# alguoo314/JASPER

Measured on AMD Instinct MI355X. Metric: assembly Mbp/s polished + Gk-mers/s counted, k=37, higher is better.
Workload: dtype u64

## Files before the change

jasper_amd/csrc/count_part.hip:

```cpp
#include "table.hpp"
#include <algorithm>
#include <cmath>
#include <cstdio>
#include <cstdlib>
#include <type_traits>
#include <vector>

namespace jk {

#define HIPCHK(x)                                                                     \
    do {                                                                              \
        hipError_t e_ = (x);                                                          \
        if (e_ != hipSuccess) {                                                       \
            err = std::string(#x) + ": " + hipGetErrorString(e_);                     \
            return -1;                                                                \
        }                                                                             \
    } while (0)

__device__ __forceinline__ void lds_barrier() { asm volatile("s_waitcnt lgkmcnt(0)\n\ts_barrier" ::: "memory"); }

constexpr int PT_THREADS = 1024;
constexpr int PT_GROUP = 16;
constexpr int PT_TILE = PT_THREADS * PT_GROUP;
constexpr int PT_HALO = 4;
// ... 686 lines not shown
                uint32_t b2;
                if constexpr (OWN) {
                    b2 = G.p2 ? (uint32_t)(rec[j] >> shift2) & ((1u << G.p2) - 1u) : 0u;
                    b2 |= owner_of(hash_of(b1, rec[j], G.recbits), nown) << G.p2;
                } else b2 = (uint32_t)(rec[j] >> shift2) & (uint32_t)(nb2 - 1);
                br[j] = (b2 << 16) | (atomicAdd(&s_cnt[b2], 1u) & 0xFFFFu);
            }
            lds_barrier();
            {
                const unsigned int v0 = 2 * t < nb2 ? s_cnt[2 * t] : 0u, v1 = 2 * t + 1 < nb2 ? s_cnt[2 * t + 1] : 0u;
                const unsigned int v = v0 + v1;
                unsigned int inc = v;
#pragma unroll
                for (int o = 1; o < 64; o <<= 1) { const unsigned int u = __shfl_up(inc, o); if ((t & 63) >= o) inc += u; }
                if ((t & 63) == 63) s_wsum[t >> 6] = inc;
                lds_barrier();
                unsigned int wbase = 0;
                for (int w = 0; w < (t >> 6); ++w) wbase += s_wsum[w];
                const unsigned int ex = wbase + inc - v;
                if (2 * t < nb2) s_off[2 * t] = ex;
                if (2 * t + 1 < nb2) s_off[2 * t + 1] = ex + v0;
                if (t == PT_THREADS - 1) s_off[nb2] = wbase + inc;
            }
            lds_barrier();
#pragma unroll
            for (int j = 0; j < PT_GROUP; ++j)
                if (br[j] != 0xFFFFFFFFu) s_stage[s_off[br[j] >> 16] + (br[j] & 0xFFFFu)] = rec[j];
            lds_barrier();
            {
                const int lpb = nb2 <= 256 ? 64 : 16;
                const int g = t / lpb, r = t % lpb;
                for (int b2 = g; b2 < nb2; b2 += PT_THREADS / lpb) {
                    const unsigned int off = s_off[b2], cnt = s_cnt[b2], cur = s_cur[b2];
                    const uint64_t region = OWN ? ((((uint64_t)(b2 >> G.p2) << G.p1) + b1) << G.p2) + (uint64_t)(b2 & ((1 << G.p2) - 1))
                                                : ((uint64_t)b1 << G.p2) + (uint64_t)b2;
                    uint64_t *dst = out2 + (region * G.nblk2 + blockIdx.x) * G.cap2;
                    for (unsigned int q = r; q < cnt; q += lpb) {
                        const unsigned int pos = cur + q;
                        const uint64_t rr = s_stage[off + q];
                        if (pos < G.cap2) dst[pos] = rr;
                        else if (MIN && cbits) {
                            const u128 hh = hash_of(b1, rr & ((1ull << G.recbits) - 1ull), G.recbits);
                            const unsigned long long di = atomicAdd(deferred_n, 1ull);
                            if (di < deferred_cap) { deferred[3 * di] = hh.hi; deferred[3 * di + 1] = hh.lo; deferred[3 * di + 2] = ((rr >> G.recbits) & ((1ull << cbits) - 1ull)) + 1ull; }
                            else atomicExch(&T.stats[ST_FATAL], 1ull);
                        } else defer_record(T, hash_of(b1, rr, G.recbits), deferred, deferred_n, deferred_cap);
                    }
                }
            }
            lds_barrier();
            for (int i = t; i < nb2; i += PT_THREADS) { s_cur[i] += s_cnt[i]; s_cnt[i] = 0; }
            lds_barrier();
        }
        for (int i = t; i < nb2; i += PT_THREADS) {
            const uint64_t region = OWN ? ((((uint64_t)(i >> G.p2) << G.p1) + b1) << G.p2) + (uint64_t)(i & ((1 << G.p2) - 1)) : ((uint64_t)b1 << G.p2) + (uint64_t)i;
            cnt2[region * G.nblk2 + blockIdx.x] = s_cur[i] < G.cap2 ? s_cur[i] : G.cap2;
        }
        lds_barrier();
    }
}
constexpr size_t P2_LDS = (size_t)PT_TILE * 8 + (size_t)(3 * PT_MAXBUCKETS + 1 + 16 + P2_MAXSL + 1) * 4;

constexpr int P2F_LINE = 16;
struct P2Meta { uint64_t gbase; uint32_t lim; int32_t cadd; };
__device__ __forceinline__ u128 rec_hash(uint64_t b1, uint64_t r, int recbits) { return hash_of(b1, r, recbits); }
__device__ __forceinline__ u128 rec_hash(uint64_t b1, Rec16 r, int recbits) { return hash_of16(b1, r, recbits); }
template <int MAXB, int ROWS, int RB = 8> struct P2F {
    static constexpr int TILE = PT_THREADS * ROWS;
    static constexpr int PIECE = 64 * ROWS * 9;
    static constexpr size_t LDS = (size_t)TILE * RB + (size_t)(3 * (MAXB + 4) + 32) * 4 + (size_t)MAXB * sizeof(P2Meta) + (size_t)MAXB * 128;
};
struct P2Args {
    int p1, p2, recbits;
    uint32_t nblk1, vper, nblk2, cap1, cap2;
    uint32_t nown;
    unsigned long long *stats;
};
template <int MAXB, int ROWS, bool OWN = false, typename REC = uint64_t>
__global__ __launch_bounds__(PT_THREADS, 4) void part2f_kernel(const REC *__restrict__ out1, const unsigned int *__restrict__ cnt1, P2Args P, REC *__restrict__ out2,
                                                            unsigned int *__restrict__ cnt2, unsigned long long *__restrict__ deferred,
                                                            unsigned long long *__restrict__ deferred_n, uint64_t deferred_cap) {
    constexpr int P2F_MAXB = MAXB, P2F_ROWS = ROWS, P2F_PIECE = P2F<MAXB, ROWS>::PIECE;
    constexpr bool W16 = sizeof(REC) == 16;
    constexpr int RB = (int)sizeof(REC), P2F_LINE = 128 / RB;
    typedef __attribute__((address_space(1))) REC global_rec;
    constexpr int NSW = MAXB / 64;
    extern __shared__ __align__(16) unsigned char s_raw[];
    P2Meta *s_meta = reinterpret_cast<P2Meta *>(s_raw);
    REC *s_carry = reinterpret_cast<REC *>(s_meta + P2F_MAXB);
    unsigned int *s_cnt = reinterpret_cast<unsigned int *>(s_carry + P2F_MAXB * P2F_LINE);
    unsigned int *s_off = s_cnt + P2F_MAXB + 4;
    unsigned int *s_have = s_off + P2F_MAXB + 4;
    unsigned int *s_wsum = s_have + P2F_MAXB + 4;
    REC *s_stage = reinterpret_cast<REC *>(s_wsum + 32);
    const int t = threadIdx.x;
    const int nb2 = OWN ? (int)(P.nown << P.p2) : 1 << P.p2;
    const int shift2 = P.recbits - P.p2;
    const uint32_t wave = (uint32_t)__builtin_amdgcn_readfirstlane(t >> 6), lane = (uint32_t)t & 63u;
    for (uint32_t b1 = blockIdx.y; b1 < (1u << P.p1); b1 += gridDim.y) {
        auto list_of = [&](uint32_t b2) -> uint64_t {
            if constexpr (OWN) return ((((uint64_t)(b2 >> P.p2) << P.p1) + b1) << P.p2) + (uint64_t)(b2 & ((1u << P.p2) - 1u));
            else return ((uint64_t)b1 << P.p2) + (uint64_t)b2;
        };
        auto b2_of = [&](REC rr) -> uint32_t {
            if constexpr (W16) return (uint32_t)shr(mk(rr.hi, rr.lo), (unsigned)shift2).lo & (uint32_t)(nb2 - 1);
            else if constexpr (OWN) {
                const uint32_t lo = P.p2 ? (uint32_t)(rr >> shift2) & ((1u << P.p2) - 1u) : 0u;
                return lo | (owner_of(hash_of(b1, rr, P.recbits), P.nown) << P.p2);
            } else return (uint32_t)(rr >> shift2) & (uint32_t)(nb2 - 1);
        };
        auto slice_of = [&](uint32_t b2) { return reinterpret_cast<uint64_t>(out2 + (list_of(b2) * P.nblk2 + blockIdx.x) * P.cap2); };
        if (t < P2F_MAXB + 4) s_cnt[t] = 0;
        if (t == 0) { s_wsum[16] = 0; s_wsum[17] = 0; }
        static_assert(P2F_MAXB + 4 <= PT_THREADS && NSW >= 1 && NSW <= 16, "list counts are scanned by the first MAXB / 64 waves");
        lds_barrier();
        auto piece_len = [&](uint32_t ph_, uint32_t sub_) -> uint32_t {
            const uint32_t c = cnt1[((uint64_t)ph_ << P.p1) + b1], first = sub_ * (uint32_t)P2F_PIECE;
            return c > first ? (c - first < (uint32_t)P2F_PIECE ? c - first : (uint32_t)P2F_PIECE) : 0u;
        };
        {
            uint32_t rounds = 0;
            for (uint32_t q = wave + 16u * lane;; q += 16u * 64u) {
                const uint32_t ph_ = blockIdx.x + P.nblk2 * (q / P.vper);
                if (ph_ >= P.nblk1) break;
                rounds += (piece_len(ph_, q % P.vper) + 64u * P2F_ROWS - 1u) / (64u * P2F_ROWS);
            }
            for (int o = 32; o > 0; o >>= 1) rounds += __shfl_xor(rounds, o);
            if (lane == 0) atomicMax(&s_wsum[17], rounds);
        }
        lds_barrier();
        const uint32_t rounds = s_wsum[17];
        uint32_t pos = 0;
        uint32_t ph = blockIdx.x + P.nblk2 * (wave / P.vper), sub = wave % P.vper;
        auto open_piece = [&](uint32_t &len_out, const REC *&src_out) {
            len_out = 0;
            if (ph < P.nblk1) {
                const uint32_t c = (uint32_t)__builtin_amdgcn_readfirstlane((int)cnt1[((uint64_t)ph << P.p1) + b1]), first = sub * (uint32_t)P2F_PIECE;
                len_out = c > first ? (c - first < (uint32_t)P2F_PIECE ? c - first : (uint32_t)P2F_PIECE) : 0u;
            }
            src_out = out1 + ((uint64_t)b1 * P.nblk1 + ph) * P.cap1 + (uint64_t)sub * P2F_PIECE;
        };
        uint32_t slen;
        const REC *src;
        open_piece(slen, src);
        unsigned int cur = 0, have = 0;
        REC rec[P2F_ROWS];
        auto fetch = [&](REC (&dst)[P2F_ROWS], uint32_t &valid) {
            while (pos >= slen && ph < P.nblk1) {
                sub += 16u;
                while (sub >= P.vper) { sub -= P.vper; ph += P.nblk2; }
                pos = 0;
                open_piece(slen, src);
            }
            valid = 0;
#pragma unroll
            for (int j = 0; j < P2F_ROWS; ++j) {
                const uint32_t i = pos + (uint32_t)j * 64u + lane;
                if constexpr (W16) { dst[j].lo = ~0ull; dst[j].hi = ~0ull; } else dst[j] = ~0ull;
                if (i < slen) { dst[j] = src[i]; valid |= 1u << j; }
            }
            pos += 64u * P2F_ROWS;
        };
        uint32_t vmask = 0;
        constexpr bool PF = true;
        REC nxt[P2F_ROWS];
        uint32_t vmask_n = 0;
        if (PF && rounds) {
            fetch(rec, vmask);
#pragma unroll
            for (int j = 0; j < P2F_ROWS; ++j) { if constexpr (W16) asm volatile("" : "+v"(rec[j].lo), "+v"(rec[j].hi)); else asm volatile("" : "+v"(rec[j])); }
        }
        for (uint32_t round = 0; round < rounds; ++round) {
            if constexpr (PF) { if (round + 1 < rounds) fetch(nxt, vmask_n); else vmask_n = 0; }
            else fetch(rec, vmask);
            uint32_t br[P2F_ROWS];
#pragma unroll
            for (int j = 0; j < P2F_ROWS; ++j) {
                const uint32_t b2 = (vmask >> j) & 1u ? b2_of(rec[j]) : (uint32_t)nb2;
                br[j] = (b2 << 16) | (atomicAdd(&s_cnt[b2], 1u) & 0xFFFFu);
            }
            lds_barrier();
            unsigned int v = 0, inc = 0;
            if (t < P2F_MAXB) {
                v = t < nb2 ? s_cnt[t] : 0u;
                inc = wave_scan_incl(v);
                if (lane == 63) s_wsum[wave] = inc;
                s_cnt[t] = 0;
                if (t == 0) s_cnt[nb2] = 0;
            }
            lds_barrier();
            unsigned int total, wbase;
            if constexpr (NSW == 2) { total = s_wsum[0] + s_wsum[1]; wbase = wave ? s_wsum[0] : 0u; }
            else {
                const unsigned int ws = wave_scan_incl(lane < (uint32_t)NSW ? s_wsum[lane] : 0u);
                wbase = wave && wave < (uint32_t)NSW ? (unsigned int)__builtin_amdgcn_readlane((int)ws, (int)wave - 1) : 0u;
                total = (unsigned int)__builtin_amdgcn_readlane((int)ws, NSW - 1);
            }
            unsigned int F = 0;
            if (t < nb2) {
                const unsigned int ex = inc - v + wbase;
                const unsigned int T = have + v;
                F = T & ~(unsigned int)(P2F_LINE - 1);
                const unsigned int L = F ? F - have : 0u;
                s_off[t] = ex;
                P2Meta M;
                M.gbase = slice_of((uint32_t)t) + ((uint64_t)cur + (uint64_t)have - (uint64_t)ex) * (uint64_t)RB;
                M.lim = ex + L;
                M.cadd = F ? -(int32_t)(ex + L) : (int32_t)have - (int32_t)ex;
                s_meta[t] = M;
                s_have[t] = have | (F ? 0x80000000u : 0u);
                if (cur + F > P.cap2) s_wsum[16] = 1;
            }
            if (t == 0) s_off[nb2] = total;
            lds_barrier();
#pragma unroll
            for (int j = 0; j < P2F_ROWS; ++j) s_stage[s_off[br[j] >> 16] + (br[j] & 0xFFFFu)] = rec[j];
            int td = t;
            asm volatile("" : "+v"(td));
            constexpr int NU = P2F_MAXB / 64;
            REC cw[NU];
            uint32_t cat[NU];
#pragma unroll
            for (int u = 0; u < NU; ++u) {
                if constexpr (W16) { cw[u].lo = 0ull; cw[u].hi = 0ull; } else cw[u] = 0ull;
                cat[u] = ~0u;
                const uint32_t b2 = ((uint32_t)td >> 4) + (uint32_t)u * 64u, q = (uint32_t)td & 15u;
                if (b2 < (uint32_t)nb2) {
                    const unsigned int hv = s_have[b2];
                    if ((hv >> 31) && q < (hv & 0xFFFFu)) {
                        cw[u] = s_carry[b2 * P2F_LINE + q];
                        const P2Meta M = s_meta[b2];
                        cat[u] = (uint32_t)((int64_t)(M.gbase - slice_of(b2)) / RB + (int64_t)s_off[b2]) - (hv & 0xFFFFu) + q;
                    }
                }
            }
            const bool overflow = s_wsum[16] != 0;
            if constexpr (PF) {
#pragma unroll
                for (int j = 0; j < P2F_ROWS; ++j) { if constexpr (W16) asm volatile("" : "+v"(nxt[j].lo), "+v"(nxt[j].hi)); else asm volatile("" : "+v"(nxt[j])); }
            }
            lds_barrier();
            if (!overflow) {
#pragma unroll
                for (int u = 0; u < NU; ++u)
                    if (cat[u] != ~0u) reinterpret_cast<global_rec *>(slice_of(((uint32_t)td >> 4) + (uint32_t)u * 64u))[cat[u]] = cw[u];
#pragma unroll 2
                for (unsigned int i = (unsigned int)td; i < total; i += PT_THREADS) {
                    const REC rr = s_stage[i];
                    const uint32_t b2 = b2_of(rr);
                    const P2Meta M = s_meta[b2];
                    if (i < M.lim) reinterpret_cast<global_rec *>(M.gbase)[i] = rr;
                    else s_carry[b2 * P2F_LINE + (uint32_t)((int32_t)i + M.cadd)] = rr;
                }
            } else {
                auto put = [&](uint32_t b2, uint64_t at, REC rr) {
                    if (at < P.cap2) reinterpret_cast<global_rec *>(slice_of(b2))[at] = rr;
                    else defer_record(P.stats, rec_hash(b1, rr, P.recbits), deferred, deferred_n, deferred_cap);
                };
#pragma unroll
                for (int u = 0; u < NU; ++u)
                    if (cat[u] != ~0u) put(((uint32_t)td >> 4) + (uint32_t)u * 64u, cat[u], cw[u]);
                for (unsigned int i = (unsigned int)td; i < total; i += PT_THREADS) {
                    const REC rr = s_stage[i];
                    const uint32_t b2 = b2_of(rr);
                    const P2Meta M = s_meta[b2];
                    if (i < M.lim) put(b2, (uint64_t)((int64_t)(M.gbase - slice_of(b2)) / RB + (int64_t)i), rr);
                    else s_carry[b2 * P2F_LINE + (uint32_t)((int32_t)i + M.cadd)] = rr;
                }
            }
            if (t < nb2) { cur += F; have = have + v - F; }
            if constexpr (PF) {
#pragma unroll
                for (int j = 0; j < P2F_ROWS; ++j) rec[j] = nxt[j];
                vmask = vmask_n;
            }
        }
        lds_barrier();
        if (t < nb2) {
            for (unsigned int q = 0; q < have; ++q) {
                const REC rr = s_carry[(uint32_t)t * P2F_LINE + q];
                if (cur + q < P.cap2) reinterpret_cast<global_rec *>(slice_of((uint32_t)t))[cur + q] = rr;
                else defer_record(P.stats, rec_hash(b1, rr, P.recbits), deferred, deferred_n, deferred_cap);
            }
            const unsigned int n = cur + have;
            cnt2[list_of((uint32_t)t) * P.nblk2 + blockIdx.x] = n < P.cap2 ? n : P.cap2;
        }
        lds_barrier();
    }
}

constexpr int LDS_HBINS = 1024;
constexpr int LI_MAXSL = 64;
__device__ __forceinline__ uint32_t scalar_load_u32(const unsigned int *p) {
    uint32_t v;
    asm volatile("s_load_dword %0, %1, 0x0\n\ts_waitcnt lgkmcnt(0)" : "=s"(v) : "s"(p) : "memory");
    return v;
}
constexpr int RI_TH = 512;
#ifndef JK_RI_PF
#define JK_RI_PF 6
#endif
constexpr int RI_PF = 8;
constexpr int RI_PF_AHEAD = JK_RI_PF;
template <bool FRESH, bool XCHG = false, typename REC = uint64_t, bool R12 = false>
__global__ __launch_bounds__(RI_TH) void region_insert_kernel(const REC *__restrict__ lists, const unsigned int *__restrict__ cnt, uint32_t cap, uint32_t nsl,
                                                              TableDev T, PartGeom G, uint32_t nregions, unsigned long long *__restrict__ deferred,
                                                              unsigned long long *__restrict__ deferred_n, uint64_t deferred_cap,
                                                              unsigned long long *__restrict__ histo, uint32_t nsrc = 1, int cbits = 0, int fbits = 0) {
    using cnt_t = typename std::conditional<FRESH && !XCHG, unsigned int, unsigned long long>::type;
    constexpr bool W16 = sizeof(REC) == 16;
    static_assert(!(W16 && XCHG), "the exchange ships 8-byte records");
    constexpr bool AHEAD = FRESH && !XCHG && R12 && !W16;
    constexpr int PF = AHEAD ? RI_PF_AHEAD : RI_PF;
    auto rec_zero = []() { REC z; if constexpr (W16) { z.lo = 0ull; z.hi = 0ull; } else z = 0ull; return z; };
    extern __shared__ __align__(16) unsigned long long s_tag[];
    const uint32_t R = 1u << G.rbits;
    cnt_t *s_cnt = reinterpret_cast<cnt_t *>(s_tag + R);
    unsigned int *s_bins = reinterpret_cast<unsigned int *>(s_cnt + R);
    unsigned int *s_pref = s_bins + LDS_HBINS;
    const int t = threadIdx.x;
    const int rs = T.B - T.s;
    const uint64_t rmask = (1ull << rs) - 1ull;
    const bool whole = nregions == 1;
    unsigned long long fresh = 0;
    if (!XCHG && deferred_n[1]) return;
    if (histo) {
        for (int i = t; i < LDS_HBINS; i += RI_TH) s_bins[i] = 0;
    }
    uint32_t region = blockIdx.x;
    uint64_t first = 0, b1 = 0;
    uint32_t nrec = 0, total = 0;
    const uint32_t per_src = XCHG ? nsl / nsrc : nsl;
    auto slice_of = [&](uint32_t x) -> uint64_t {
        if constexpr (XCHG) return ((uint64_t)(x / per_src) * nregions + region) * per_src + x % per_src;
        else return (uint64_t)region * nsl + x;
    };
    auto count_of = [&](uint32_t region_, uint32_t x_) -> uint32_t {
        if constexpr (AHEAD) return scalar_load_u32(cnt + ((uint64_t)region_ * nsl + x_));
        else return cnt[(uint64_t)region_ * nsl + x_];
    };
    REC recs[PF], recs2[PF];
    auto fetch = [&](REC (&dst)[PF], uint32_t region_, uint32_t x_, uint32_t i0_, uint32_t n_) {
        const REC *s = lists + ((uint64_t)region_ * nsl + x_) * cap;
#pragma unroll
        for (int u = 0; u < PF; ++u) {
            const uint32_t i = i0_ + (uint32_t)u * RI_TH + t;
            if constexpr (AHEAD) dst[u] = s[i < n_ ? i : 0u];
            else dst[u] = i < n_ ? s[i] : rec_zero();
        }
    };
    auto probe_on = [&](REC rec, uint32_t idx, unsigned long long want, unsigned long long cur, cnt_t inc) {
        for (;;) {
            if (cur == 0ull) {
                cur = atomicCAS(&s_tag[idx], 0ull, want);
                if (cur == 0ull) { ++fresh; cur = want; }
            }
            if (cur == want) { atomicAdd(&s_cnt[idx], inc); return; }
            ++idx;
            ++want;
            if (whole) idx &= R - 1;
            if (idx >= R || (want & (unsigned long long)(MAXPROBE - 1)) == 0ull) {
                if constexpr (XCHG) {
                    const u128 hh = hash_of(b1, rec, G.recbits);
                    const unsigned long long di = atomicAdd(deferred_n, 1ull);
                    if (di < deferred_cap) { deferred[3 * di] = hh.hi; deferred[3 * di + 1] = hh.lo; deferred[3 * di + 2] = (unsigned long long)inc; }
                    else atomicExch(&T.stats[ST_FATAL], 1ull);
                } else defer_record(T, rec_hash(b1, rec, G.recbits), deferred, deferred_n, deferred_cap);
                return;
            }
            cur = s_tag[idx];
        }
    };
    auto insert_batch = [&](REC (&rr)[PF], uint32_t i0, uint32_t n) {
        uint32_t idx[PF];
        unsigned long long want[PF], cur[PF];
        cnt_t inc[PF];
#pragma unroll
        for (int u = 0; u < PF; ++u) {
            inc[u] = (cnt_t)1;
            if constexpr (XCHG) {
                if (cbits) {
                    const int csh = G.recbits - fbits;
                    const uint64_t fmask = ((1ull << fbits) - 1ull) << csh;
                    inc[u] = (cnt_t)(((rr[u] >> csh) & ((1ull << cbits) - 1ull)) + 1ull);
                    rr[u] = (rr[u] & ~fmask) | ((uint64_t)((region >> (G.p2 - fbits)) & ((1u << fbits) - 1u)) << csh);
                }
            }
            if constexpr (W16) {
                idx[u] = (uint32_t)shr(mk(rr[u].hi, rr[u].lo), (unsigned)rs).lo & (R - 1);
                want[u] = OCC | ((rr[u].lo & rmask) << OFFBITS);
            } else {
                idx[u] = (uint32_t)(rr[u] >> rs) & (R - 1);
                want[u] = OCC | ((rr[u] & rmask) << OFFBITS);
            }
            cur[u] = s_tag[idx[u]];
        }
#pragma unroll
        for (int u = 0; u < PF; ++u) {
            if (i0 + (uint32_t)u * RI_TH + t < n) {
                if (cur[u] == want[u]) atomicAdd(&s_cnt[idx[u]], inc[u]);
                else probe_on(rr[u], idx[u], want[u], cur[u], inc[u]);
            }
        }
    };
    auto open_region = [&]() -> bool {
        first = (uint64_t)region << G.rbits;
        b1 = region >> G.p2;
        if constexpr (XCHG) {
            total = 0;
            for (uint32_t x = 0; x < nsl; ++x) total += cnt[slice_of(x)];
            if (!FRESH && !histo && !total) return false;
            if (t == 0) {
                unsigned int run = 0;
                for (uint32_t x = 0; x < nsl; ++x) { s_pref[x] = run; run += cnt[slice_of(x)]; }
                s_pref[nsl] = run;
            }
        } else {
            nrec = count_of(region, 0u);
            if (!FRESH && !histo) {
                uint32_t any = nrec;
                for (uint32_t x = 1; x < nsl; ++x) any |= count_of(region, x);
                if (!any) return false;
            }
        }
        return true;
    };
    auto image_setup = [&]() {
        if (FRESH) {
            for (uint32_t i = t; i < R; i += RI_TH) { s_tag[i] = 0ull; s_cnt[i] = 0; }
        } else {
            for (uint32_t i = t; i < R; i += RI_TH) {
                const ulonglong2 e = *reinterpret_cast<const ulonglong2 *>(T.slots + 2 * (first + i));
                s_tag[i] = e.x;
                s_cnt[i] = (cnt_t)e.y;
            }
        }
    };
    auto insert_region = [&]() {
        if constexpr (XCHG) {
            uint32_t x = 0;
            for (uint32_t i0 = 0; i0 < total; i0 += PF * RI_TH) {
#pragma unroll
                for (int u = 0; u < PF; ++u) {
                    const uint32_t i = i0 + (uint32_t)u * RI_TH + t;
                    recs[u] = rec_zero();
                    if (i < total) {
                        while (s_pref[x + 1] <= i) ++x;
                        recs[u] = lists[slice_of(x) * cap + (i - s_pref[x])];
                    }
                }
                insert_batch(recs, i0, total);
            }
        } else {
            uint32_t x = 0, i0 = 0;
            auto advance = [&]() -> bool {
                i0 += PF * RI_TH;
                while (x < nsl && i0 >= nrec) { ++x; i0 = 0; nrec = x < nsl ? count_of(region, x) : 0u; }
                return x < nsl;
            };
            if constexpr (AHEAD) {
                for (;;) {
                    const uint32_t ia = i0, na = nrec;
                    const bool more_b = advance();
                    fetch(recs2, region, more_b ? x : 0u, more_b ? i0 : 0u, nrec);
                    insert_batch(recs, ia, na);
                    if (!more_b) break;
                    const uint32_t ib = i0, nb_ = nrec;
                    const bool more_a = advance();
                    fetch(recs, region, more_a ? x : 0u, more_a ? i0 : 0u, nrec);
                    insert_batch(recs2, ib, nb_);
                    if (!more_a) break;
                }
#pragma unroll
                for (int u = 0; u < PF; ++u) asm volatile("" :: "v"(recs[u]), "v"(recs2[u]));
            } else {
                for (;;) {
                    insert_batch(recs, i0, nrec);
                    if (!advance()) break;
                    fetch(recs, region, x, i0, nrec);
                }
            }
        }
    };
    auto write_slot = [&](uint32_t i) {
        const unsigned long long tag = s_tag[i];
        const unsigned long long c64 = (unsigned long long)s_cnt[i];
        *reinterpret_cast<ulonglong2 *>(T.slots + 2 * (first + i)) = make_ulonglong2(tag, c64);
        if (histo) {
            const bool occ = tag != 0ull && c64 != 0ull;
            const uint32_t c = clamp32(c64);
            const uint32_t b = c > 10001u ? 10001u : c;
            const unsigned long long ones = __ballot(occ && b == 1u);
            if (ones && (t & 63) == (int)__builtin_ctzll(ones)) atomicAdd(&s_bins[1], (unsigned int)__popcll(ones));
            if (occ && b != 1u) {
                if (b < (uint32_t)LDS_HBINS) atomicAdd(&s_bins[b], 1u);
                else atomicAdd(&histo[b], 1ull);
            }
        }
    };
    auto write_region = [&]() {
        if constexpr (R12) {
            static_assert(!R12 || (1 << 12) == 8 * RI_TH, "eight slots per lane");
#pragma unroll
            for (int j = 0; j < 8; ++j) write_slot((uint32_t)t + (uint32_t)j * RI_TH);
        } else
            for (uint32_t i = t; i < R; i += RI_TH) write_slot(i);
    };
    if constexpr (AHEAD) {
        if (region < nregions) {
            open_region();
            fetch(recs, region, 0u, 0u, nrec);
            image_setup();
            lds_barrier();
            insert_region();
            for (;;) {
                const uint32_t next = region + gridDim.x;
                const bool has_next = next < nregions;
                const uint32_t n_next = has_next ? count_of(next, 0u) : 0u;
                fetch(recs, has_next ? next : region, 0u, 0u, n_next);
                lds_barrier();
                write_region();
                lds_barrier();
                if (!has_next) break;
                region = next;
                open_region();
                image_setup();
                lds_barrier();
                insert_region();
            }
        }
    } else {
        for (; region < nregions; region += gridDim.x) {
            if (!open_region()) continue;
            if constexpr (!XCHG) fetch(recs, region, 0u, 0u, nrec);
            image_setup();
            lds_barrier();
            insert_region();
            lds_barrier();
            write_region();
            lds_barrier();
        }
    }
    if (histo) {
        for (int i = t; i < LDS_HBINS; i += RI_TH)
            if (s_bins[i]) atomicAdd(&histo[i], (unsigned long long)s_bins[i]);
    }
    for (int o = 32; o > 0; o >>= 1) fresh += __shfl_xor(fresh, o);
    lds_barrier();
    if (t == 0) s_tag[0] = 0ull;
    lds_barrier();
    if ((t & 63) == 0 && fresh) atomicAdd(&s_tag[0], fresh);
    lds_barrier();
    if (t == 0 && s_tag[0]) atomicAdd(&T.stats[ST_DISTINCT], s_tag[0]);
}

constexpr int RIW_PF = 4;
template <bool FRESH>
__global__ __launch_bounds__(RI_TH) void region_insertw_kernel(const Rec16 *__restrict__ lists, const unsigned int *__restrict__ cnt, uint32_t cap, uint32_t nsl, TableDev T,
                                                               PartGeom G, uint32_t nregions, unsigned long long *__restrict__ deferred,
                                                               unsigned long long *__restrict__ deferred_n, uint64_t deferred_cap) {
    using cnt_t = typename std::conditional<FRESH, unsigned int, unsigned long long>::type;
    extern __shared__ __align__(16) unsigned long long s_tag[];
    const uint32_t R = 1u << G.rbits;
    unsigned long long *s_ext = s_tag + R;
    cnt_t *s_cnt = reinterpret_cast<cnt_t *>(s_ext + R);
    const int t = threadIdx.x;
    const int rs = T.B - T.s;
    const bool whole = nregions == 1;
    unsigned long long fresh = 0;
    if (deferred_n[1]) return;
    for (uint32_t region = blockIdx.x; region < nregions; region += gridDim.x) {
        const uint64_t first = (uint64_t)region << G.rbits;
        const uint64_t b1 = region >> G.p2;
        if (!FRESH) {
            uint32_t any = 0;
            for (uint32_t x = 0; x < nsl; ++x) any |= cnt[(uint64_t)region * nsl + x];
            if (!any) continue;
        }
        if (FRESH) {
            for (uint32_t i = t; i < R; i += RI_TH) { s_tag[i] = 0ull; s_ext[i] = 0ull; s_cnt[i] = 0; }
        } else {
            for (uint32_t i = t; i < R; i += RI_TH) {
                const ulonglong2 e = *reinterpret_cast<const ulonglong2 *>(T.slots + 2 * (first + i));
                s_tag[i] = e.x;
                s_cnt[i] = (cnt_t)e.y;
                s_ext[i] = T.ext[first + i];
            }
        }
        lds_barrier();
        for (uint32_t x = 0; x < nsl; ++x) {
            const uint32_t nrec = cnt[(uint64_t)region * nsl + x];
            const Rec16 *src = lists + ((uint64_t)region * nsl + x) * cap;
            for (uint32_t i0 = 0; i0 < nrec; i0 += RIW_PF * RI_TH) {
                Rec16 recs[RIW_PF];
#pragma unroll
                for (int u = 0; u < RIW_PF; ++u) {
                    const uint32_t i = i0 + (uint32_t)u * RI_TH + t;
                    recs[u].lo = 0ull; recs[u].hi = 0ull;
                    if (i < nrec) recs[u] = src[i];
                }
#pragma unroll
                for (int u = 0; u < RIW_PF; ++u) {
                    const u128 rr = mk(recs[u].hi, recs[u].lo);
                    uint32_t idx = (uint32_t)shr(rr, (unsigned)rs).lo & (R - 1);
                    const u128 rem = band(rr, maskbits((unsigned)rs));
                    unsigned long long want = OCC | (rem.hi << OFFBITS);
                    const unsigned long long ext = rem.lo;
                    bool done = !(i0 + (uint32_t)u * RI_TH + t < nrec);
                    uint32_t waited = 0;
                    for (;;) {
                        if (!done) {
                            unsigned long long cur = __hip_atomic_load(&s_tag[idx], __ATOMIC_RELAXED, __HIP_MEMORY_SCOPE_WORKGROUP);
                            if (cur == 0ull) {
                                cur = atomicCAS(&s_tag[idx], 0ull, want);
                                if (cur == 0ull) {
                                    __hip_atomic_store(&s_ext[idx], ext, __ATOMIC_RELAXED, __HIP_MEMORY_SCOPE_WORKGROUP);
                                    __hip_atomic_fetch_add(&s_cnt[idx], (cnt_t)1, __ATOMIC_RELEASE, __HIP_MEMORY_SCOPE_WORKGROUP);
                                    ++fresh;
                                    done = true;
                                }
                            }
                            if (!done) {
                                bool next = true;
                                if (cur == want) {
                                    const cnt_t c = __hip_atomic_load(&s_cnt[idx], __ATOMIC_ACQUIRE, __HIP_MEMORY_SCOPE_WORKGROUP);
                                    if (c == 0) {
                                        next = false;
                                        if (++waited > (1u << 16)) { defer_record(T, hash_of16(b1, recs[u], G.recbits), deferred, deferred_n, deferred_cap); done = true; }
                                    } else if (__hip_atomic_load(&s_ext[idx], __ATOMIC_RELAXED, __HIP_MEMORY_SCOPE_WORKGROUP) == ext) {
                                        __hip_atomic_fetch_add(&s_cnt[idx], (cnt_t)1, __ATOMIC_RELAXED, __HIP_MEMORY_SCOPE_WORKGROUP);
                                        done = true;
                                    }
                                }
                                if (!done && next) {
                                    ++idx;
                                    ++want;
                                    if (whole) idx &= R - 1;
                                    if (idx >= R || (want & (unsigned long long)(MAXPROBE - 1)) == 0ull) {
                                        defer_record(T, hash_of16(b1, recs[u], G.recbits), deferred, deferred_n, deferred_cap);
                                        done = true;
                                    }
                                }
                            }
                        }
                        if (__ballot(!done) == 0ull) break;
                    }
                }
            }
        }
        lds_barrier();
        for (uint32_t i = t; i < R; i += RI_TH) {
            *reinterpret_cast<ulonglong2 *>(T.slots + 2 * (first + i)) = make_ulonglong2(s_tag[i], (unsigned long long)s_cnt[i]);
            T.ext[first + i] = s_ext[i];
        }
        lds_barrier();
    }
    for (int o = 32; o > 0; o >>= 1) fresh += __shfl_xor(fresh, o);
    if ((threadIdx.x & 63) == 0 && fresh) atomicAdd(&T.stats[ST_DISTINCT], fresh);
}

__global__ __launch_bounds__(256) void import3w_kernel(const unsigned long long *__restrict__ entries, const unsigned long long *__restrict__ n_ptr, uint64_t cap, TableDev T) {
    if (n_ptr[1]) return;
    const uint64_t n = *n_ptr < cap ? *n_ptr : cap;
    unsigned long long fresh = 0;
    for (uint64_t i0 = (blockIdx.x * (uint64_t)blockDim.x + threadIdx.x) & ~63ull; i0 < n; i0 += (uint64_t)gridDim.x * blockDim.x) {
        const uint64_t i = i0 + (threadIdx.x & 63);
        int r = 1;
        if (i < n) r = table_add(T, mk(entries[3 * i], entries[3 * i + 1]), entries[3 * i + 2]);
        if (r == 2) ++fresh;
        if (r == 0) table_spill(T, mk(entries[3 * i], entries[3 * i + 1]), entries[3 * i + 2]);
    }
    for (int o = 32; o > 0; o >>= 1) fresh += __shfl_xor(fresh, o);
    if ((threadIdx.x & 63) == 0 && fresh) atomicAdd(&T.stats[ST_DISTINCT], fresh);
}

__global__ void part_decide_kernel(unsigned long long *__restrict__ deferred_n, uint64_t deferred_cap, const unsigned long long *__restrict__ stats) {
    if (deferred_n[0] > deferred_cap || stats[ST_FATAL]) deferred_n[1] = 1ull;
}

__device__ __forceinline__ uint32_t histo_bin(unsigned long long c) { const uint32_t v = clamp32(c); return v > 10001u ? 10001u : v; }
__global__ __launch_bounds__(256) void import3h_kernel(const unsigned long long *__restrict__ entries, const unsigned long long *__restrict__ n_ptr, uint64_t cap,
                                                       TableDev T, unsigned long long *__restrict__ histo) {
    if (n_ptr[1]) return;
    const uint64_t n = *n_ptr < cap ? *n_ptr : cap;
    unsigned long long fresh = 0;
    constexpr int NB = 64;
    __shared__ int s_delta[NB];
    if (threadIdx.x < NB) s_delta[threadIdx.x] = 0;
    __syncthreads();
    for (uint64_t i0 = (blockIdx.x * (uint64_t)blockDim.x + threadIdx.x) & ~63ull; i0 < n; i0 += (uint64_t)gridDim.x * blockDim.x) {
        const uint64_t i = i0 + (threadIdx.x & 63);
        const bool have = i < n;
        u128 h = mk(0, 0);
        unsigned long long inc = 0;
        if (have) { h = mk(entries[3 * i], entries[3 * i + 1]); inc = entries[3 * i + 2]; }
        {
            const int lead = (int)__builtin_ctzll(__ballot(have));
            const uint64_t lhi = (uint64_t)__shfl((long long)h.hi, lead), llo = (uint64_t)__shfl((long long)h.lo, lead);
            const bool same = have && h.hi == lhi && h.lo == llo;
            unsigned long long part = same ? inc : 0ull;
            for (int o = 32; o > 0; o >>= 1) part += (unsigned long long)__shfl_xor((long long)part, o);
            if (same) inc = (int)(threadIdx.x & 63) == lead ? part : 0ull;
        }
        if (!have || !inc) continue;
        const uint64_t home = home_of(h, T.B, T.s);
        const uint64_t rem = rem_of(h, T.B, T.s);
// ... 562 lines not shown
```

Before: 3149.

## Restructure region insert into grouped hit pass plus wave-uniform probe loop

The region insert batch now decodes and looks up LDS tags in small groups (HG) separated by scheduling barriers, which limits live registers. Hits are applied with an unconditional atomicAdd that adds zero to an idle slot on misses, so no branch is needed. Misses are recorded in a pending bitmask and resolved in a single ballot-driven loop that walks one record per lane at a time, replacing the per-record divergent probe loop. Each miss is decoded a second time in exchange for less divergence and lower register pressure, and every lane issues an extra LDS atomic even when it has no hit.

Result: slower. 3092 (-1.8%).

```diff
diff --git a/jasper_amd/csrc/count_part.hip b/jasper_amd/csrc/count_part.hip
--- a/jasper_amd/csrc/count_part.hip
+++ b/jasper_amd/csrc/count_part.hip
@@ -1012,6 +1012,10 @@
 #endif
 constexpr int RI_PF = 8;
 constexpr int RI_PF_AHEAD = JK_RI_PF;
+#ifndef JK_RI_HG
+#define JK_RI_HG 3
+#endif
+constexpr int RI_HG_AHEAD = JK_RI_HG;
 template <bool FRESH, bool XCHG = false, typename REC = uint64_t, bool R12 = false>
 __global__ __launch_bounds__(RI_TH) void region_insert_kernel(const REC *__restrict__ lists, const unsigned int *__restrict__ cnt, uint32_t cap, uint32_t nsl,
                                                               TableDev T, PartGeom G, uint32_t nregions, unsigned long long *__restrict__ deferred,
@@ -1022,6 +1026,7 @@
     static_assert(!(W16 && XCHG), "the exchange ships 8-byte records");
     constexpr bool AHEAD = FRESH && !XCHG && R12 && !W16;
     constexpr int PF = AHEAD ? RI_PF_AHEAD : RI_PF;
+    constexpr int HG = AHEAD ? RI_HG_AHEAD : PF;
     auto rec_zero = []() { REC z; if constexpr (W16) { z.lo = 0ull; z.hi = 0ull; } else z = 0ull; return z; };
     extern __shared__ __align__(16) unsigned long long s_tag[];
     const uint32_t R = 1u << G.rbits;
@@ -1050,68 +1055,119 @@
         else return cnt[(uint64_t)region_ * nsl + x_];
     };
     REC recs[PF], recs2[PF];
+    auto lane_base = [&](uint32_t i0_) -> uint32_t {
+        uint32_t v = i0_ + (uint32_t)t;
+        asm("" : "+v"(v));
+        return v;
+    };
     auto fetch = [&](REC (&dst)[PF], uint32_t region_, uint32_t x_, uint32_t i0_, uint32_t n_) {
         const REC *s = lists + ((uint64_t)region_ * nsl + x_) * cap;
+        const uint32_t ibase = lane_base(i0_);
 #pragma unroll
         for (int u = 0; u < PF; ++u) {
-            const uint32_t i = i0_ + (uint32_t)u * RI_TH + t;
+            const uint32_t i = ibase + (uint32_t)u * RI_TH;
             if constexpr (AHEAD) dst[u] = s[i < n_ ? i : 0u];
             else dst[u] = i < n_ ? s[i] : rec_zero();
         }
     };
-    auto probe_on = [&](REC rec, uint32_t idx, unsigned long long want, unsigned long long cur, cnt_t inc) {
-        for (;;) {
-            if (cur == 0ull) {
-                cur = atomicCAS(&s_tag[idx], 0ull, want);
-                if (cur == 0ull) { ++fresh; cur = want; }
-            }
-            if (cur == want) { atomicAdd(&s_cnt[idx], inc); return; }
-            ++idx;
-            ++want;
-            if (whole) idx &= R - 1;
-            if (idx >= R || (want & (unsigned long long)(MAXPROBE - 1)) == 0ull) {
-                if constexpr (XCHG) {
-                    const u128 hh = hash_of(b1, rec, G.recbits);
-                    const unsigned long long di = atomicAdd(deferred_n, 1ull);
-                    if (di < deferred_cap) { deferred[3 * di] = hh.hi; deferred[3 * di + 1] = hh.lo; deferred[3 * di + 2] = (unsigned long long)inc; }
-                    else atomicExch(&T.stats[ST_FATAL], 1ull);
-                } else defer_record(T, rec_hash(b1, rec, G.recbits), deferred, deferred_n, deferred_cap);
-                return;
-            }
-            cur = s_tag[idx];
+    auto decode = [&](REC raw, REC &rec, uint32_t &idx, unsigned long long &want, cnt_t &inc) {
+        rec = raw;
+        inc = (cnt_t)1;
+        if constexpr (XCHG) {
+            if (cbits) {
+                const int csh = G.recbits - fbits;
+                const uint64_t fmask = ((1ull << fbits) - 1ull) << csh;
+                inc = (cnt_t)(((raw >> csh) & ((1ull << cbits) - 1ull)) + 1ull);
+                rec = (raw & ~fmask) | ((uint64_t)((region >> (G.p2 - fbits)) & ((1u << fbits) - 1u)) << csh);
+            }
+        }
+        if constexpr (W16) {
+            idx = (uint32_t)shr(mk(rec.hi, rec.lo), (unsigned)rs).lo & (R - 1);
+            want = OCC | ((rec.lo & rmask) << OFFBITS);
+        } else {
+            idx = (uint32_t)(rec >> rs) & (R - 1);
+            want = OCC | ((rec & rmask) << OFFBITS);
         }
     };
+    const uint32_t idle_slot = R12 ? (uint32_t)t : (uint32_t)t & (R - 1);
     auto insert_batch = [&](REC (&rr)[PF], uint32_t i0, uint32_t n) {
-        uint32_t idx[PF];
-        unsigned long long want[PF], cur[PF];
-        cnt_t inc[PF];
-#pragma unroll
-        for (int u = 0; u < PF; ++u) {
-            inc[u] = (cnt_t)1;
-            if constexpr (XCHG) {
-                if (cbits) {
-                    const int csh = G.recbits - fbits;
-                    const uint64_t fmask = ((1ull << fbits) - 1ull) << csh;
-                    inc[u] = (cnt_t)(((rr[u] >> csh) & ((1ull << cbits) - 1ull)) + 1ull);
-                    rr[u] = (rr[u] & ~fmask) | ((uint64_t)((region >> (G.p2 - fbits)) & ((1u << fbits) - 1u)) << csh);
-                }
-            }
-            if constexpr (W16) {
-                idx[u] = (uint32_t)shr(mk(rr[u].hi, rr[u].lo), (unsigned)rs).lo & (R - 1);
-                want[u] = OCC | ((rr[u].lo & rmask) << OFFBITS);
-            } else {
-                idx[u] = (uint32_t)(rr[u] >> rs) & (R - 1);
-                want[u] = OCC | ((rr[u] & rmask) << OFFBITS);
-            }
-            cur[u] = s_tag[idx[u]];
-        }
-#pragma unroll
-        for (int u = 0; u < PF; ++u) {
-            if (i0 + (uint32_t)u * RI_TH + t < n) {
-                if (cur[u] == want[u]) atomicAdd(&s_cnt[idx[u]], inc[u]);
-                else probe_on(rr[u], idx[u], want[u], cur[u], inc[u]);
-            }
-        }
+        uint32_t pend = 0;
+        {
+            const uint32_t ibase = lane_base(i0);
+#pragma unroll
+            for (int g = 0; g < PF; g += HG) {
+                uint32_t idx[HG];
+                unsigned long long want[HG], cur[HG];
+                cnt_t inc[HG];
+#pragma unroll
+                for (int v = 0; v < HG; ++v) {
+                    if (g + v < PF) {
+                        REC rec;
+                        decode(rr[g + v], rec, idx[v], want[v], inc[v]);
+                        cur[v] = s_tag[idx[v]];
+                    }
+                }
+#pragma unroll
+                for (int v = 0; v < HG; ++v) {
+                    if (g + v < PF) {
+                        const bool valid = ibase + (uint32_t)(g + v) * RI_TH < n;
+                        const bool hit = valid & (cur[v] == want[v]);
+                        atomicAdd(&s_cnt[hit ? idx[v] : idle_slot], hit ? inc[v] : (cnt_t)0);
+                        pend |= (valid & !hit) ? 1u << (g + v) : 0u;
+                    }
+                }
+                if (g + HG < PF) __builtin_amdgcn_sched_barrier(0);
+            }
+        }
+        auto lowest = [&]() -> REC {
+            REC raw = rr[PF - 1];
+#pragma unroll
+            for (int u = PF - 2; u >= 0; --u) {
+                if (pend & (1u << u)) raw = rr[u];
+                if constexpr (W16) asm("" : "+v"(raw.lo), "+v"(raw.hi));
+                else asm("" : "+v"(raw));
+            }
+            return raw;
+        };
+        constexpr uint32_t NONE = ~0u;
+        uint32_t idx = NONE, claimed = 0;
+        unsigned long long want = 0;
+        cnt_t inc = 0;
+        while (__ballot(pend != 0u)) {
+            if (pend) {
+                if (idx == NONE) {
+                    REC rec;
+                    decode(lowest(), rec, idx, want, inc);
+                }
+                unsigned long long cur = s_tag[idx];
+                if (cur == 0ull) {
+                    cur = atomicCAS(&s_tag[idx], 0ull, want);
+                    if (cur == 0ull) { ++claimed; cur = want; }
+                }
+                bool done = cur == want;
+                if (done) atomicAdd(&s_cnt[idx], inc);
+                else {
+                    ++idx;
+                    ++want;
+                    if (whole) idx &= R - 1;
+                    if (idx >= R || (want & (unsigned long long)(MAXPROBE - 1)) == 0ull) {
+                        REC rec;
+                        uint32_t idx0;
+                        unsigned long long want0;
+                        decode(lowest(), rec, idx0, want0, inc);
+                        if constexpr (XCHG) {
+                            const u128 hh = hash_of(b1, rec, G.recbits);
+                            const unsigned long long di = atomicAdd(deferred_n, 1ull);
+                            if (di < deferred_cap) { deferred[3 * di] = hh.hi; deferred[3 * di + 1] = hh.lo; deferred[3 * di + 2] = (unsigned long long)inc; }
+                            else atomicExch(&T.stats[ST_FATAL], 1ull);
+                        } else defer_record(T, rec_hash(b1, rec, G.recbits), deferred, deferred_n, deferred_cap);
+                        done = true;
+                    }
+                }
+                if (done) { pend &= pend - 1u; idx = NONE; }
+            }
+        }
+        fresh += claimed;
     };
     auto open_region = [&]() -> bool {
         first = (uint64_t)region << G.rbits;
```
